# nateraw/stable-diffusion-videos

Hardware: NVIDIA H100
Metric: frames/sec at 512x512 50-step SD-1.4 (higher is better)
Workload: dtype f16

## Files before the change

### include/sdwalk.h

```cpp
#ifndef SDWALK_H_
#define SDWALK_H_

#include <stdint.h>

#ifdef __cplusplus
extern "C" {
#endif

#define SDW_ABI_VERSION 2

const char* sdw_last_error(void);
int sdw_abi_version(void);
void sdw_debug_plan_only(int on);

int sdw_slerp_lerp_batch(const void* lat_a, const void* lat_b, const void* emb_a, const void* emb_b,
                         const float* t, int n_frames, int64_t n_lat, int64_t n_emb, int dtype_is_f16,
                         float dot_threshold, void* out_lat, void* out_emb, void* stream);

typedef struct sdw_step_coef {
  float guidance;
  float c_x;
  float c_e[5];
  int32_t hist_slot[4];
  int32_t use_x_base;
// ... 61 lines not shown
int sdw_engine_debug_profile(sdw_engine* e, const char* path, void* stream);

typedef struct sdw_gemm_desc {
  const void* A;
  int32_t C, W, H, B;
  int64_t sW, sH, sB;
  int32_t conv;
  int32_t up_px, up_py;
  const void* Wt;
  int32_t N;
  int64_t ldb, Kb;
  int32_t b_batched;
  int64_t sBh, sBb;
  const float* bias;
  const float* rowvec;
  int32_t rowvec_ld;
  const void* resid;
  int64_t ldr;
  void* out;
  int64_t ldc;
  int64_t o_sW, o_sH, o_sB;
  int32_t mode;
  int32_t act;
  float alpha;
  int32_t vt_col0, vt_d, vt_heads, vt_ntok;
  void* vt;
  int64_t vt_ld;
  int32_t bn;
  int32_t ver;
  int32_t nsub;
  int32_t ew;
  int32_t tr;
  int32_t et;
  int32_t reserved0;
} sdw_gemm_desc;

int sdw_gemm(const sdw_gemm_desc* desc, void* stream);
int sdw_debug_plan(const sdw_gemm_desc* desc, int32_t out[12]);

int sdw_attention(const void* q, int64_t q_ld, const void* k, int64_t k_ld, const void* vt, int64_t vt_ld, int B,
                  int Nq, int Nk, int heads, int d, void* out, int64_t out_ld, void* stream);

int sdw_groupnorm(const void* x, int64_t ldx, int B, int64_t P, int C, int G, const float* gamma, const float* beta,
                  float eps, int silu, void* y, int64_t ldy, void* stream);
int sdw_layernorm(const void* x, int64_t ldx, int64_t rows, int C, const float* gamma, const float* beta, float eps,
                  void* y, int64_t ldy, void* stream);

int sdw_softmax_rows(void* s, int64_t ld, int64_t rows, int n, void* stream);
int sdw_conv_in_small(const void* x, int64_t ldx, int B, int H, int W, int Cin, const void* w, const float* bias, int N,
                      void* y, int64_t ldy, void* stream);
int sdw_conv_out_small(const void* x, int64_t ldx, int B, int H, int W, int C, const void* w, const float* bias, int nout,
                       float* out_f32, uint8_t* out_u8, void* stream);
int sdw_vae_in(const float* x, float inv_scale, const void* w, const float* bias, int F, int C, int H, int W, void* z,
               void* stream);
int sdw_timestep_embed(const float* t, int n, int dim, int round_f16, float* out, void* stream);
int sdw_linear_f32(const float* in, int64_t ldi, const void* w, const float* bias, int M, int N, int K, int silu_in,
                   int silu_out, float* out, int64_t ldo, void* stream);
int sdw_wrap_pad(const void* x, int64_t ld_bytes, int B, int H, int W, int pix_bytes, int pad, void* y, void* stream);
int sdw_crop_interior(const void* yp, int B, int H, int W, int pix_bytes, int crop, const void* resid_f16, int64_t ldr,
                      void* out, int64_t ldo_bytes, void* stream);

int sdw_debug_attention_plan(int B, int Nq, int Nk, int heads, int d, int32_t out[5]);

int sdw_pack_weight(const void* w_oihw, int N, int C, int kh, int kw, int geglu_interleave, void* out, void* stream);
int sdw_pack_weight_up4(const void* w_oihw, int N, int C, void* out, void* stream);

typedef struct sdw_clip sdw_clip;
// ... 54 lines not shown
```

### stable-diffusion-videos_b200/_native.py

```python
import ctypes as C
import os

import torch

_HERE = os.path.dirname(os.path.abspath(__file__))
LIB_PATH = os.path.join(_HERE, "libsdwalk.so")
_lib = None


class SdwError(RuntimeError):
    pass


class StepCoef(C.Structure):
    _fields_ = [
        ("guidance", C.c_float), ("c_x", C.c_float), ("c_e", C.c_float * 5),
        ("hist_slot", C.c_int32 * 4), ("use_x_base", C.c_int32), ("save_x_base", C.c_int32),
        ("push_slot", C.c_int32), ("next_in_scale", C.c_float), ("push_e", C.c_float), ("push_x", C.c_float),
    ]


class GemmDesc(C.Structure):
    _fields_ = [
        ("A", C.c_void_p), ("C", C.c_int32), ("W", C.c_int32), ("H", C.c_int32), ("B", C.c_int32),
        ("sW", C.c_int64), ("sH", C.c_int64), ("sB", C.c_int64),
        ("conv", C.c_int32), ("up_px", C.c_int32), ("up_py", C.c_int32),
        ("Wt", C.c_void_p), ("N", C.c_int32), ("ldb", C.c_int64), ("Kb", C.c_int64),
        ("b_batched", C.c_int32), ("sBh", C.c_int64), ("sBb", C.c_int64),
        ("bias", C.c_void_p), ("rowvec", C.c_void_p), ("rowvec_ld", C.c_int32),
        ("resid", C.c_void_p), ("ldr", C.c_int64),
        ("out", C.c_void_p), ("ldc", C.c_int64),
        ("o_sW", C.c_int64), ("o_sH", C.c_int64), ("o_sB", C.c_int64),
        ("mode", C.c_int32), ("act", C.c_int32), ("alpha", C.c_float),
        ("vt_col0", C.c_int32), ("vt_d", C.c_int32), ("vt_heads", C.c_int32), ("vt_ntok", C.c_int32),
        ("vt", C.c_void_p), ("vt_ld", C.c_int64), ("bn", C.c_int32), ("ver", C.c_int32), ("nsub", C.c_int32), ("ew", C.c_int32), ("tr", C.c_int32), ("et", C.c_int32), ("reserved0", C.c_int32),
    ]


def lib():
    global _lib
    if _lib is None:
        if not os.path.exists(LIB_PATH):
            raise SdwError(
                f"{LIB_PATH} not built: run `python __graft_entry__.py build` "
                "(the native sm_90a library is required; there is no fallback path)")
        _lib = C.CDLL(LIB_PATH)
        _lib.sdw_last_error.restype = C.c_char_p
    return _lib


def check(rc):
    if rc != 0:
        raise SdwError(f"libsdwalk error {rc}: {lib().sdw_last_error().decode()}")


def stream_ptr():
    return C.c_void_p(torch.cuda.current_stream().cuda_stream)


def ptr(t):
    return C.c_void_p(t.data_ptr()) if t is not None else C.c_void_p(0)


def require_cuda(*tensors):
    for t in tensors:
        if t is not None and not t.is_cuda:
            raise SdwError("libsdwalk operates on CUDA tensors only (no CPU fallback)")

# ... 129 lines not shown
```

### stable-diffusion-videos_b200/csrc/sdw_capi.cu

```cuda
#include "../../include/sdwalk.h"
#include "sdw_internal.h"

#include <cstdlib>
#include <cstring>

namespace sdw {
static thread_local std::string g_err;
void set_error(const std::string& msg) { g_err = msg; }
bool pdl_enabled() {
  static const bool on = [] { const char* e = std::getenv("SDW_PDL"); return e && e[0] == '1'; }();
  return on;
}
const char* last_error() { return g_err.c_str(); }
}

using namespace sdw;

extern "C" {

const char* sdw_last_error(void) { return sdw::last_error(); }
int sdw_abi_version(void) { return SDW_ABI_VERSION; }
void sdw_debug_plan_only(int on) { sdw::set_plan_only(on != 0); }

int sdw_slerp_lerp_batch(const void* lat_a, const void* lat_b, const void* emb_a, const void* emb_b, const float* t,
                         int n_frames, int64_t n_lat, int64_t n_emb, int dtype_is_f16, float dot_threshold,
                         void* out_lat, void* out_emb, void* stream) {
  return slerp_lerp_batch(lat_a, lat_b, emb_a, emb_b, t, n_frames, n_lat, n_emb, dtype_is_f16, dot_threshold,
                          out_lat, out_emb, static_cast<cudaStream_t>(stream));
}

int sdw_cfg_sched_step(const void* eps_nhwc, int has_uncond, float* x, float* x_base, float* hist,
                       const sdw_step_coef* coef, int F, int C, int H, int W, void* next_in, int next_in_cpad,
                       void* stream) {
  return cfg_sched_step(static_cast<const float*>(eps_nhwc), has_uncond, x, x_base, hist, coef, F, C, H, W, next_in,
                        next_in_cpad, static_cast<cudaStream_t>(stream));
}

int sdw_latents_init(const void* latents, int dtype_is_f16, float init_noise_sigma, float in_scale, float* x,
                     void* model_in, int model_in_cpad, int dup, int F, int C, int H, int W, void* stream) {
  return latents_init(latents, dtype_is_f16, init_noise_sigma, in_scale, x, model_in, model_in_cpad, dup, F, C, H, W,
                      static_cast<cudaStream_t>(stream));
}

static int to_desc(const sdw_gemm_desc* c, GemmDesc& d);

int sdw_debug_plan(const sdw_gemm_desc* c, int32_t out[12]) {
  SDW_REQUIRE(c != nullptr && out != nullptr, "null");
  GemmDesc d;
  if (int e = to_desc(c, d)) return e;
  GemmLaunch L;
  if (int e = plan_gemm(d, &L)) return e;
  out[0] = L.ver; out[1] = L.bn; out[2] = L.nsub; out[3] = L.ew; out[4] = L.tr;
  out[5] = L.p.epi_tma; out[6] = L.p.nstages; out[7] = 0;
  out[8] = static_cast<int32_t>(L.grid.x); out[9] = L.p.bw; out[10] = L.p.bh; out[11] = L.p.bb;
  return 0;
}

int sdw_gemm(const sdw_gemm_desc* c, void* stream) {
  SDW_REQUIRE(c != nullptr, "null desc");
  GemmDesc d;
  if (int e = to_desc(c, d)) return e;
  GemmLaunch L;
  if (int e = plan_gemm(d, &L)) return e;
  return launch_gemm(L, static_cast<cudaStream_t>(stream));
}

static int to_desc(const sdw_gemm_desc* c, GemmDesc& d) {
  d.A = static_cast<const __half*>(c->A);
  d.C = c->C; d.W = c->W; d.H = c->H; d.B = c->B;
  d.sW = c->sW; d.sH = c->sH; d.sB = c->sB;
  d.conv = c->conv; d.up_px = c->up_px; d.up_py = c->up_py;
  d.Wt = static_cast<const __half*>(c->Wt);
  d.N = c->N; d.ldb = c->ldb; d.Kb = c->Kb;
  d.b_batched = c->b_batched; d.sBh = c->sBh; d.sBb = c->sBb;
  d.bias = c->bias; d.rowvec = c->rowvec; d.rowvec_ld = c->rowvec_ld;
  d.resid = static_cast<const __half*>(c->resid); d.ldr = c->ldr;
  d.out = static_cast<__half*>(c->out); d.ldc = c->ldc;
  d.o_sW = c->o_sW; d.o_sH = c->o_sH; d.o_sB = c->o_sB;
  d.mode = c->mode; d.act = c->act; d.alpha = c->alpha;
  d.vt_col0 = c->vt_col0; d.vt_d = c->vt_d; d.vt_heads = c->vt_heads; d.vt_ntok = c->vt_ntok;
  d.vt = static_cast<__half*>(c->vt); d.vt_ld = c->vt_ld;
  d.bn = c->bn;
  d.ver = c->ver;
  d.nsub = c->nsub;
  d.ew = c->ew;
  d.tr = c->tr;
  d.et = c->et;
  return 0;
}

int sdw_attention(const void* q, int64_t q_ld, const void* k, int64_t k_ld, const void* vt, int64_t vt_ld, int B,
                  int Nq, int Nk, int heads, int d, void* out, int64_t out_ld, void* stream) {
  AttnDesc a;
  a.q = static_cast<const __half*>(q); a.q_ld = q_ld;
  a.k = static_cast<const __half*>(k); a.k_ld = k_ld;
  a.vt = static_cast<const __half*>(vt); a.vt_ld = vt_ld;
  a.B = B; a.Nq = Nq; a.Nk = Nk; a.heads = heads; a.d = d;
  a.out = static_cast<__half*>(out); a.out_ld = out_ld;
  AttnLaunch L;
  if (int e = plan_attention(a, &L)) return e;
  return launch_attention(L, static_cast<cudaStream_t>(stream));
}

int sdw_groupnorm(const void* x, int64_t ldx, int B, int64_t P, int C, int G, const float* gamma, const float* beta,
                  float eps, int silu, void* y, int64_t ldy, void* stream) {
  cudaStream_t st = static_cast<cudaStream_t>(stream);
  float2* ws = nullptr;
  SDW_CUDA_OK(cudaMallocAsync(&ws, gn_workspace_bytes(B), st));
  const int rc = groupnorm(static_cast<const __half*>(x), ldx, B, P, C, G, gamma, beta, eps, silu, static_cast<__half*>(y),
                           ldy, ws, st);
  cudaFreeAsync(ws, st);
  return rc;
}

int sdw_layernorm(const void* x, int64_t ldx, int64_t rows, int C, const float* gamma, const float* beta, float eps,
                  void* y, int64_t ldy, void* stream) {
  return layernorm(static_cast<const __half*>(x), ldx, rows, C, gamma, beta, eps, static_cast<__half*>(y), ldy,
                   static_cast<cudaStream_t>(stream));
}

// ... 67 lines not shown
```

### stable-diffusion-videos_b200/csrc/sdw_gemm.cu

```cuda
#include "sdw_internal.h"
#include "sdw_ptx.cuh"

#include <cudaTypedefs.h>

#include <algorithm>
#include <cstdlib>
#include <cstring>

namespace sdw {

static constexpr int BM = 128;
static constexpr int BK = 64;
static constexpr int GEMM_THREADS = 288;
static constexpr int A_STAGE = BM * BK * 2;
static constexpr int TR_BW = 16, TR_BH = 8;
static constexpr int A_STAGE_TR = (TR_BH + 2) * TR_BW * 128;

template <int BN, int NSUB, int TR>
struct GemmCfg {
  static constexpr int A_BYTES = TR ? A_STAGE_TR : A_STAGE;
  static constexpr int TAPS = TR ? 3 : 1;
  static constexpr int B_SUB = BN * 128;
  static constexpr int B_BYTES = TAPS * NSUB * B_SUB;
};

struct EpiRow {
  bool ok;
  int64_t out_off, res_off, pix;
  const float* rowvec;
};

template <int BN, int XE>
__device__ __forceinline__ void gemm_epilogue(const GemmKParams& p, float (&acc)[BN / 2], int n_base, const EpiRow (&R)[2],
                                              int lane, int wg, int lrow0, uint8_t* stage, uint64_t* res_full, int x0,
                                              int y0, int b0, uint32_t& chunk_count) {
  const int q2 = 2 * (lane & 3);
  const bool vec2 = p.vec2;
  const bool use_tma = p.epi_tma;
  const int r0 = 64 * wg;
  const int tx = x0 + (r0 & (p.bw - 1)), ty = y0 + ((r0 >> p.lg_bw) & (p.bh - 1)), tb = b0 + (r0 >> (p.lg_bw + p.lg_bh));
  const bool issuer = (threadIdx.x & 127) == 0;
  const bool tma_res = use_tma && p.resid != nullptr;
  const int nch = (min(BN, p.N - n_base) + 31) >> 5;
  auto res_issue = [&](int c, uint32_t k) {
    if (tma_res && issuer && c < nch) {
      mbar_expect_tx(&res_full[k & 1], 4096);
      tma_load_4d(&p.mapRes, &res_full[k & 1], stage + (k & 1) * 4096, n_base + 32 * c, tx, ty, tb);
    }
  };
  if (tma_res && p.mode == GEMM_PLAIN) {
    if (issuer) bulk_wait_group_read<1>();
    res_issue(0, chunk_count);
  }

  auto value = [&](float v, int n, int h) {
    float o = v * p.alpha;
    if (p.bias) o += __ldg(p.bias + n);
    if (p.rowvec) o += __ldg(R[h].rowvec + n);
    if (p.act == 1) o = silu_f(o);
    if constexpr (XE != 0) {
      if (p.act == 2) o = o > 0.f ? o : 0.2f * o;
    }
    return o;
  };
  auto add_res = [&](float& o, float r) {
    if constexpr (XE != 0) o = fmaf(p.res_scale, r, o);
    else o += r;
  };
  auto plain_pair = [&](int j, int n, uint8_t* staged, int scol) {
#pragma unroll
    for (int h = 0; h < 2; ++h) {
      float o0 = n < p.N ? value(acc[4 * j + 2 * h], n, h) : 0.f;
// ... 9 lines not shown
          add_res(o0, f.x);
          add_res(o1, f.y);
          if (XE != 0 && p.resid2) {
            const float2 g = __half22float2(*reinterpret_cast<const __half2*>(p.resid2 + R[h].res_off + n));
            o0 += g.x;
            o1 += g.y;
          }
        } else {
          if (n < p.N) add_res(o0, __half2float(p.resid[R[h].res_off + n]));
          if (n + 1 < p.N) add_res(o1, __half2float(p.resid[R[h].res_off + n + 1]));
          if (XE != 0 && p.resid2) {
            if (n < p.N) o0 += __half2float(p.resid2[R[h].res_off + n]);
            if (n + 1 < p.N) o1 += __half2float(p.resid2[R[h].res_off + n + 1]);
          }
        }
      }
      if (staged) {
        *reinterpret_cast<uint32_t*>(staged + (lrow0 + 8 * h) * 64 + scol * 2) = pack_h2(o0, o1);
      } else if (R[h].ok) {
        __half* dst = p.out + R[h].out_off + n;
        if (vec2 && n + 1 < p.N) {
          *reinterpret_cast<uint32_t*>(dst) = pack_h2(o0, o1);
        } else {
          if (n < p.N) dst[0] = __float2half_rn(o0);
          if (n + 1 < p.N) dst[1] = __float2half_rn(o1);
        }
      }
    }
  };
  auto vt_pair = [&](int j, int n) {
#pragma unroll
    for (int h = 0; h < 2; ++h) {
      if (!R[h].ok) continue;
      const int64_t bq = R[h].pix / p.vt_ntok;
      const int tok = static_cast<int>(R[h].pix - bq * p.vt_ntok);
#pragma unroll
      for (int e = 0; e < 2; ++e) {
        const int nn = n + e;
        if (nn >= p.N) continue;
        float o = acc[4 * j + 2 * h + e] * p.alpha;
        if (p.bias) o += __ldg(p.bias + nn);
        const int cc = nn - p.vt_col0, head = cc / p.vt_d, dd = cc - head * p.vt_d;
        p.vt[((bq * p.vt_heads + head) * p.vt_d + dd) * p.vt_ld + tok] = __float2half_rn(o);
      }
    }
  };
  auto stage_begin = [&]() {
    if (issuer) bulk_wait_group_read<1>();
    asm volatile("bar.sync %0, 128;" ::"r"(1 + wg) : "memory");
    return stage + (chunk_count & 1) * 4096;
  };
  auto stage_end = [&](uint8_t* buf, int col) {
    fence_proxy_async_smem();
    asm volatile("bar.sync %0, 128;" ::"r"(1 + wg) : "memory");
    if (issuer) {
      tma_store_4d(&p.mapOut, buf, col, tx, ty, tb);
      bulk_commit_group();
    }
    ++chunk_count;
  };

  if (p.mode == GEMM_GEGLU) {
#pragma unroll
    for (int c = 0; c < BN / 64; ++c) {
      const int n = n_base + 64 * c;
      if (n >= p.N) break;
      uint8_t* buf = use_tma ? stage_begin() : nullptr;
#pragma unroll
      for (int jj = 0; jj < 4; ++jj) {
        const int j = 8 * c + jj;
        const int na = n + 8 * jj + q2, ng = na + 32;
        float o[2][2];
#pragma unroll
        for (int h = 0; h < 2; ++h)
#pragma unroll
          for (int e = 0; e < 2; ++e) {
// ... 20 lines not shown
          }
        }
      }
      if (use_tma) stage_end(buf, n / 2);
    }
    return;
  }
#pragma unroll
  for (int c = 0; c < BN / 32; ++c) {
    const int n = n_base + 32 * c;
    if (n >= p.N) break;
    if (p.mode == GEMM_QKV_VT && n >= p.vt_col0) {
#pragma unroll
      for (int jj = 0; jj < 4; ++jj) vt_pair(4 * c + jj, n + 8 * jj + q2);
      continue;
    }
    if (use_tma) {
      uint8_t* buf = stage_begin();
      if (tma_res) {
        if (issuer && c + 1 < nch) bulk_wait_group_read<0>();
        res_issue(c + 1, chunk_count + 1);
        mbar_wait(&res_full[chunk_count & 1], (chunk_count >> 1) & 1);
      }
#pragma unroll
      for (int jj = 0; jj < 4; ++jj) plain_pair(4 * c + jj, n + 8 * jj + q2, buf, 8 * jj + q2);
      stage_end(buf, n);
    } else {
#pragma unroll
      for (int jj = 0; jj < 4; ++jj) plain_pair(4 * c + jj, n + 8 * jj + q2, nullptr, 0);
    }
  }
}

template <int BN, int NSUB, int TR, int CL, int XE>
__global__ void __launch_bounds__(GEMM_THREADS, 1) gemm_kernel(const __grid_constant__ GemmKParams p) {
  using Cfg = GemmCfg<BN, NSUB, TR>;
  constexpr int A_BYTES = Cfg::A_BYTES;
  constexpr int B_BYTES = Cfg::B_BYTES;
  const int STAGES = p.nstages;
  extern __shared__ uint8_t smem_raw[];
  uint8_t* smem = reinterpret_cast<uint8_t*>((reinterpret_cast<uintptr_t>(smem_raw) + 1023) & ~uintptr_t(1023));
  uint64_t* full_bar = reinterpret_cast<uint64_t*>(smem);
  uint64_t* empty_bar = full_bar + GEMM_MAX_STAGES;
  uint8_t* smem_a = smem + GEMM_BAR_BYTES;
  uint8_t* smem_b = smem_a + STAGES * A_BYTES;
  uint8_t* epi_stage = smem_b + STAGES * B_BYTES;
  uint64_t* res_full = empty_bar + GEMM_MAX_STAGES;

  const int warp = threadIdx.x >> 5, lane = threadIdx.x & 31;
  const uint32_t rank = CL > 1 ? cluster_ctarank() : 0;
  const int cluster_id = blockIdx.x / CL;
  const int nclusters = gridDim.x / CL;
  const int total_tiles = p.m_groups * p.n_tiles;
  const int num_kb = TR ? 3 * p.kchunks : p.ntaps * p.kchunks;

  if (warp == 8 && lane == 0) {
    tma_prefetch_desc(&p.mapA[0]);
    tma_prefetch_desc(&p.mapB);
    if (p.epi_tma) tma_prefetch_desc(&p.mapOut);
    for (int s = 0; s < STAGES; ++s) {
      mbar_init(&full_bar[s], 1);
      mbar_init(&empty_bar[s], 2 * CL);
    }
    for (int i = 0; i < 4; ++i) mbar_init(&res_full[i], 1);
    if (p.epi_tma && p.resid) tma_prefetch_desc(&p.mapRes);
    fence_barrier_init();
  }
  if (CL > 1) cluster_sync_all();
  else __syncthreads();
  pdl_wait();
  pdl_launch_dependents();

  auto tile_coords = [&](int t, int& x0, int& y0, int& b0, int& n0) {
    const int m_group = t / p.n_tiles;
    const int n_tile = t - m_group * p.n_tiles;
    const int m_tile = m_group * CL + static_cast<int>(rank);
    const int twh = p.tiles_w * p.tiles_h;
    const int tb = m_tile / twh;
    const int rem = m_tile - tb * twh;
    const int th = rem / p.tiles_w;
    const int tw = rem - th * p.tiles_w;
    x0 = tw * p.bw;
    y0 = th * p.bh;
    b0 = tb * p.bb;
    n0 = n_tile * (NSUB * BN);
  };

  if (warp == 8) {
    if (lane == 0) {
      int stage = 0;
      uint32_t phase = 0;
      for (int t = cluster_id; t < total_tiles; t += nclusters) {
        int x0, y0, b0, n0;
        tile_coords(t, x0, y0, b0, n0);
        int tap = 0, kc = 0;
        for (int kb = 0; kb < num_kb; ++kb) {
          mbar_wait(&empty_bar[stage], phase ^ 1);
          mbar_expect_tx(&full_bar[stage], A_BYTES + B_BYTES);
          uint8_t* a_dst = smem_a + stage * A_BYTES;
          uint8_t* b_dst = smem_b + stage * B_BYTES + rank * (BN / CL) * 128;
          const int nrow = n0 + static_cast<int>(rank) * (BN / CL);
          if (TR) {
            const int kx = tap;
            tma_load_4d(&p.mapA[0], &full_bar[stage], a_dst, kc * BK, x0 + kx - 1, y0 - 1, b0);
          } else {
            tma_load_4d(&p.mapA[p.tap_map[tap]], &full_bar[stage], a_dst, kc * BK, x0 + p.tap_dx[tap], y0 + p.tap_dy[tap],
                        b0);
          }
#pragma unroll
          for (int ky = 0; ky < Cfg::TAPS; ++ky)
#pragma unroll
            for (int sub = 0; sub < NSUB; ++sub) {
              const int kcoord = TR ? ((ky * 3 + tap) * p.kchunks + kc) * BK : kb * BK;
              uint8_t* dst = b_dst + (ky * NSUB + sub) * Cfg::B_SUB;
              const int c2 = p.b_batched ? y0 : 0, c3 = p.b_batched ? b0 : 0;
              if (CL > 1)
                tma_load_4d_mc(&p.mapB, &full_bar[stage], dst, kcoord, nrow + sub * BN, c2, c3, (1u << CL) - 1);
              else
                tma_load_4d(&p.mapB, &full_bar[stage], dst, kcoord, nrow + sub * BN, c2, c3);
            }
          if (++stage == STAGES) {
            stage = 0;
            phase ^= 1;
          }
          if (TR) {
            if (++tap == 3) {
              tap = 0;
              ++kc;
            }
          } else if (++kc == p.kchunks) {
            kc = 0;
            ++tap;
          }
        }
      }
    }
  } else {
    const int wg = warp >> 2;
    const int lrow0 = 16 * (warp & 3) + (lane >> 2);
    uint8_t* stage_buf = epi_stage + wg * 8192;
    uint32_t chunk_count = 0;
    auto release = [&](int s) {
      if ((threadIdx.x & 127) == 0) {
        if (CL > 1) {
#pragma unroll
          for (int r = 0; r < CL; ++r) mbar_arrive_cluster(mapa_rank(smem_u32(&empty_bar[s]), r));
        } else {
          mbar_arrive(&empty_bar[s]);
        }
      }
    };
    int stage = 0;
    uint32_t phase = 0;
    float acc[NSUB][BN / 2];
    for (int t = cluster_id; t < total_tiles; t += nclusters) {
      int x0, y0, b0, n0;
      tile_coords(t, x0, y0, b0, n0);
#pragma unroll
      for (int sub = 0; sub < NSUB; ++sub)
#pragma unroll
        for (int i = 0; i < BN / 2; ++i) acc[sub][i] = 0.f;
      int prev = -1;
      for (int kb = 0; kb < num_kb; ++kb) {
        mbar_wait(&full_bar[stage], phase);
        const uint32_t a_base = smem_u32(smem_a + stage * A_BYTES);
        const uint32_t b_base = smem_u32(smem_b + stage * B_BYTES);
        wgmma_fence();
#pragma unroll
        for (int ky = 0; ky < Cfg::TAPS; ++ky) {
          const uint32_t a_off = TR ? (4 * wg + ky) * (TR_BW * 128) : wg * (64 * 128);
          const uint64_t da = make_desc_k_sw128(a_base + a_off);
#pragma unroll
          for (int k = 0; k < BK / 16; ++k)
#pragma unroll
            for (int sub = 0; sub < NSUB; ++sub) {
              const uint64_t db = make_desc_k_sw128(b_base + (ky * NSUB + sub) * Cfg::B_SUB);
              Wgmma<BN>::ss(acc[sub], da + 2 * k, db + 2 * k, (kb | ky | k) != 0 ? 1u : 0u);
            }
        }
        wgmma_commit();
        wgmma_wait<1>();
        if (prev >= 0) release(prev);
        prev = stage;
        if (++stage == STAGES) {
          stage = 0;
          phase ^= 1;
        }
      }
      wgmma_wait<0>();
#pragma unroll
      for (int sub = 0; sub < NSUB; ++sub) reg_fence(acc[sub]);
      release(prev);

      EpiRow R[2];
#pragma unroll
      for (int h = 0; h < 2; ++h) {
        const int r = 64 * wg + lrow0 + 8 * h;
        const int x = x0 + (r & (p.bw - 1)), y = y0 + ((r >> p.lg_bw) & (p.bh - 1)), b = b0 + (r >> (p.lg_bw + p.lg_bh));
        R[h].ok = x < p.W && y < p.H && b < p.B;
        R[h].pix = (static_cast<int64_t>(b) * p.H + y) * p.W + x;
        const int64_t oyy = static_cast<int64_t>(y) * p.os + p.oy, oxx = static_cast<int64_t>(x) * p.os + p.ox;
        R[h].out_off = static_cast<int64_t>(b) * p.o_sB + oyy * p.o_sH + oxx * p.o_sW;
        R[h].res_off = static_cast<int64_t>(b) * p.r_sB + oyy * p.r_sH + oxx * p.r_sW;
        R[h].rowvec = p.rowvec ? p.rowvec + static_cast<int64_t>(b) * p.rowvec_ld : nullptr;
      }
#pragma unroll
      for (int sub = 0; sub < NSUB; ++sub)
        gemm_epilogue<BN, XE>(p, acc[sub], n0 + sub * BN, R, lane, wg, lrow0, stage_buf, res_full + 2 * wg, x0, y0, b0,
                          chunk_count);
    }
    if (p.epi_tma && (threadIdx.x & 127) == 0) bulk_wait_group<0>();
  }

  if (CL > 1) cluster_sync_all();
}

static PFN_cuTensorMapEncodeTiled_v12000 g_encode = nullptr;
static bool g_plan_only = false;
void set_plan_only(bool on) { g_plan_only = on; }

int sm_count() {
  static int n = 0;
  if (g_plan_only) return H100_SMS;
  if (n == 0) {
    int dev = 0;
    if (cudaGetDevice(&dev) != cudaSuccess || cudaDeviceGetAttribute(&n, cudaDevAttrMultiProcessorCount, dev) != cudaSuccess ||
        n <= 0) {
      (void)cudaGetLastError();
      n = H100_SMS;
    }
  }
  return n;
}

int gemm_init() {
  if (g_encode || g_plan_only) return 0;
  void* fn = nullptr;
  cudaDriverEntryPointQueryResult qres;
  SDW_CUDA_OK(cudaGetDriverEntryPoint("cuTensorMapEncodeTiled", &fn, cudaEnableDefault, &qres));
  if (qres != cudaDriverEntryPointSuccess || !fn) {
    set_error("cuTensorMapEncodeTiled driver entry point not available");
    return 2;
// ... 203 lines not shown
    const int groups = (m_tiles_f + CL - 1) / CL;
    for (int i = 0; i < 4; ++i) {
      const int c = cand[i];
      if (d.mode == GEMM_GEGLU && c % 64 != 0) continue;
      if (stages_for(c, 1, reuse, epi_bytes) < 2) continue;
      const int tiles = groups * ((d.N + c - 1) / c);
      const int waves = (tiles + nsm / CL - 1) / (nsm / CL);
      double cost = static_cast<double>(waves) * c;
      if (stages_for(c, 1, reuse, epi_bytes) < 3) cost *= 1.6;
      if (cost < best) {
        best = cost;
        bn = c;
      }
    }
  }
  SDW_REQUIRE(bn == 32 || bn == 64 || bn == 128 || bn == 160 || bn == 256 || (bn == 192 && ver == 2), "unsupported BLOCK_N");
  if (ver == 2) SDW_REQUIRE(bn != 32 && bn != 64, "the CTA-pair kernel needs BLOCK_N >= 128");
  if (d.ew == 4) SDW_REQUIRE(false, "one epilogue form on this GPU: epilogue width 4 is not available");
  SDW_REQUIRE(d.ew == 0 || d.ew == 2, "epilogue width must be 0 (auto) or 2");
  L->ew = 2;
  L->ver = ver;
  L->nsub = nsub;
  L->bn = bn;
  if (d.mode == GEMM_GEGLU) SDW_REQUIRE(bn % 64 == 0 && d.N % 64 == 0, "GEGLU needs 64-column pairs");
  if (d.mode == GEMM_QKV_VT) SDW_REQUIRE(d.vt && d.vt_col0 % 32 == 0 && d.vt_d > 0, "bad V^T split");
  p.nstages = stages_for(bn, nsub, reuse, epi_bytes);
  SDW_REQUIRE(p.nstages >= 2, "no room for a two-stage operand pipeline");
  p.m_groups = (m_tiles_f + CL - 1) / CL;
  p.n_tiles = (d.N + bn * nsub - 1) / (bn * nsub);
  {
    const int64_t total = static_cast<int64_t>(p.m_groups) * p.n_tiles;
    SDW_REQUIRE(total < (int64_t(1) << 31), "tile grid too large");
    L->grid = dim3(static_cast<unsigned>(CL * std::min<int64_t>(total, nsm / CL)), 1, 1);
  }
  {
    auto lg2 = [](int v) { int l = 0; while ((1 << l) < v) ++l; return l; };
    p.lg_bw = lg2(p.bw);
    p.lg_bh = lg2(p.bh);
    SDW_REQUIRE((1 << p.lg_bw) == p.bw && (1 << p.lg_bh) == p.bh, "tile extents must be powers of two");
  }
  for (int m = 0; m < nmaps; ++m) {
    const __half* base = d.A;
    uint64_t dims[4] = {static_cast<uint64_t>(d.C), static_cast<uint64_t>(d.W), static_cast<uint64_t>(d.H),
                        static_cast<uint64_t>(d.B)};
    uint64_t strides[4] = {1, static_cast<uint64_t>(d.sW), static_cast<uint64_t>(d.sH), static_cast<uint64_t>(d.sB)};
    if (d.conv == 2) {
      const int py = m / 2, px = m % 2;
      base = d.A + py * d.sH + px * d.sW;
      dims[1] = Wd;
      dims[2] = Hd;
      strides[1] = 2 * d.sW;
      strides[2] = 2 * d.sH;
    }
    for (int i = 1; i < 4; ++i)
      if (strides[i] == 0) strides[i] = static_cast<uint64_t>(Cp);
    uint32_t box[4] = {BK, static_cast<uint32_t>(bw), static_cast<uint32_t>(reuse ? bh + 2 : bh), static_cast<uint32_t>(bb)};
    if (int e = encode_map(&p.mapA[m], base, 4, dims, strides, box)) return e;
  }
  {
    const int64_t ldb = d.ldb ? d.ldb : static_cast<int64_t>(p.ntaps) * Cp;
    uint64_t dims[4] = {static_cast<uint64_t>(d.Kb ? d.Kb : static_cast<int64_t>(p.ntaps) * Cp),
                        static_cast<uint64_t>(d.N), static_cast<uint64_t>(d.b_batched ? Hd : 1),
                        static_cast<uint64_t>(d.b_batched ? d.B : 1)};
    uint64_t strides[4] = {1, static_cast<uint64_t>(ldb), static_cast<uint64_t>(d.b_batched ? d.sBh : 0),
                           static_cast<uint64_t>(d.b_batched ? d.sBb : 0)};
    for (int i = 2; i < 4; ++i)
// ... 16 lines not shown
      for (int i = 2; i < 4; ++i)
        if (sr[i] == 0 || sr[i] % 8 != 0) sr[i] = sr[1] * static_cast<uint64_t>(Wd);
      if (int e = encode_map(&p.mapRes, d.resid + p.oy * res_sH + p.ox * res_sW, 4, dims, sr, box, 0)) return e;
    }
  }
  p.bias = d.bias;
  p.rowvec = d.rowvec;
  p.rowvec_ld = d.rowvec_ld;
  p.resid = d.resid;
  p.res_scale = d.res_scale;
  p.resid2 = d.resid2;
  p.out = d.out;
  p.o_sW = osW;
  p.o_sH = osH;
  p.o_sB = osB;
  p.r_sW = res_sW;
  p.r_sH = res_sH;
  p.r_sB = res_sB;
  p.vec2 = ((p.o_sW | p.o_sH | p.o_sB) & 1) == 0 && (reinterpret_cast<uintptr_t>(d.out) & 3) == 0 &&
           (!d.resid || (((p.r_sW | p.r_sH | p.r_sB) & 1) == 0 && (reinterpret_cast<uintptr_t>(d.resid) & 3) == 0)) &&
           (!d.resid2 || (reinterpret_cast<uintptr_t>(d.resid2) & 3) == 0);
  p.mode = d.mode;
  p.act = d.act;
  p.alpha = d.alpha;
  p.vt_col0 = d.vt_col0;
  p.vt_d = d.vt_d;
  p.vt_heads = d.vt_heads;
  p.vt_ntok = d.vt_ntok > 0 ? d.vt_ntok : 1;
  p.vt = d.vt;
  p.vt_ld = d.vt_ld;
  return 0;
}

template <int BN, int NSUB, int TR, int CL, int XE = 0>
static int launch_one(const GemmLaunch& l, cudaStream_t stream) {
  static int max_ctas = 0;
  if (!max_ctas) {
    SDW_CUDA_OK(cudaFuncSetAttribute(gemm_kernel<BN, NSUB, TR, CL, XE>, cudaFuncAttributeMaxDynamicSharedMemorySize,
                                     GEMM_SMEM_DYN));
    max_ctas = sm_count();
    if (CL > 1) {
      cudaLaunchConfig_t cfg{};
      cfg.gridDim = dim3(CL * (sm_count() / CL));
      cfg.blockDim = dim3(GEMM_THREADS);
      cfg.dynamicSmemBytes = GEMM_SMEM_DYN;
      cudaLaunchAttribute attr[1];
      attr[0].id = cudaLaunchAttributeClusterDimension;
      attr[0].val.clusterDim.x = CL;
      attr[0].val.clusterDim.y = 1;
      attr[0].val.clusterDim.z = 1;
      cfg.attrs = attr;
      cfg.numAttrs = 1;
      int nclusters = 0;
      SDW_CUDA_OK(cudaOccupancyMaxActiveClusters(&nclusters, gemm_kernel<BN, NSUB, TR, CL, XE>, &cfg));
      if (nclusters > 0) max_ctas = std::min(max_ctas, CL * nclusters);
    }
  }
  const dim3 grid(std::min<unsigned>(l.grid.x, static_cast<unsigned>(max_ctas)), 1, 1);
  SDW_CUDA_OK(launch_cluster(gemm_kernel<BN, NSUB, TR, CL, XE>, grid, dim3(GEMM_THREADS), GEMM_SMEM_DYN, stream, CL, l.p));
  SDW_CUDA_OK(cudaGetLastError());
  return 0;
}

int launch_gemm(const GemmLaunch& l, cudaStream_t stream) {
  const int key = l.xe * 1000000 + l.ver * 100000 + l.bn * 100 + l.nsub * 10 + (l.tr ? 1 : 0);
  switch (key) {
    case 1103210: return launch_one<32, 1, 0, 1, 1>(l, stream);
    case 1106410: return launch_one<64, 1, 0, 1, 1>(l, stream);
    case 106410: return launch_one<64, 1, 0, 1>(l, stream);
    case 112810: return launch_one<128, 1, 0, 1>(l, stream);
    case 116010: return launch_one<160, 1, 0, 1>(l, stream);
    case 125610: return launch_one<256, 1, 0, 1>(l, stream);
    case 212810: return launch_one<128, 1, 0, 2>(l, stream);
    case 216010: return launch_one<160, 1, 0, 2>(l, stream);
    case 219210: return launch_one<192, 1, 0, 2>(l, stream);
    case 225610: return launch_one<256, 1, 0, 2>(l, stream);
    case 216020: return launch_one<160, 2, 0, 2>(l, stream);
    case 212811: return launch_one<128, 1, 1, 2>(l, stream);
    case 216011: return launch_one<160, 1, 1, 2>(l, stream);
    case 219211: return launch_one<192, 1, 1, 2>(l, stream);
    case 225611: return launch_one<256, 1, 1, 2>(l, stream);
    case 216021: return launch_one<160, 2, 1, 2>(l, stream);
    default: break;
  }
  set_error("no GEMM kernel for this version / BLOCK_N / accumulators / tap reuse combination");
  return 1;
}

}
```

### stable-diffusion-videos_b200/csrc/sdw_internal.h

```cpp
#pragma once
#include <cuda.h>
#include <cuda_fp16.h>
#include <cuda_runtime.h>
#include <stdint.h>

#include <cstdio>
#include <functional>
#include <string>
#include <unordered_map>
#include <vector>

namespace sdw {

void set_error(const std::string& msg);
const char* last_error();
#define SDW_CUDA_OK(expr)                                                                      \
  do {                                                                                         \
    cudaError_t _e = (expr);                                                                   \
    if (_e != cudaSuccess) {                                                                   \
      (void)cudaGetLastError();  \
      ::sdw::set_error(std::string(#expr) + ": " + cudaGetErrorString(_e));                    \
      return 2;                                                                                \
    }                                                                                          \
  } while (0)
// ... 69 lines not shown
  int m_groups, n_tiles;
  int N;
  int b_batched;
  int epi_tma;
  int nstages;
  int vec2;
  const float* bias;
  const float* rowvec;
  int rowvec_ld;
  const __half* resid;
  int64_t r_sW, r_sH, r_sB;
  float res_scale;
  const __half* resid2;
  __half* out;
  int64_t o_sW, o_sH, o_sB;
  int os, ox, oy;
  int mode;
  int act;
  float alpha;
  int vt_col0, vt_d, vt_heads, vt_ntok;
  __half* vt;
  int64_t vt_ld;
};

struct GemmLaunch {
  GemmKParams p;
  dim3 grid;
  int bn;
  int ver;
  int nsub = 1;
  int ew = 2;
  int tr = 0;
  int xe = 0;
};

struct GemmDesc {
  const __half* A = nullptr;
  int C = 0, W = 0, H = 1, B = 1;
  int64_t sW = 0, sH = 0, sB = 0;
  int conv = 0;
  int up_px = 0, up_py = 0;
  const __half* Wt = nullptr;
  int N = 0;
  int64_t ldb = 0;
  int64_t Kb = 0;
  int b_batched = 0;
  int64_t sBh = 0, sBb = 0;
  const float* bias = nullptr;
  const float* rowvec = nullptr;
  int rowvec_ld = 0;
  const __half* resid = nullptr;
  int64_t ldr = 0;
  int64_t r_sW = 0, r_sH = 0, r_sB = 0;
  float res_scale = 1.f;
  const __half* resid2 = nullptr;
  __half* out = nullptr;
  int64_t ldc = 0;
  int64_t o_sW = 0, o_sH = 0, o_sB = 0;
  int mode = GEMM_PLAIN;
  int act = 0;
  float alpha = 1.f;
  int vt_col0 = 0, vt_d = 0, vt_heads = 0, vt_ntok = 0;
  __half* vt = nullptr;
  int64_t vt_ld = 0;
  int bn = 0;
  int ver = 0;
  int nsub = 0;
  int ew = 0;
  int tr = 0;
  int et = 0;
};

int plan_gemm(const GemmDesc& d, GemmLaunch* out);
int launch_gemm(const GemmLaunch& l, cudaStream_t stream);
void set_plan_only(bool on);
int gemm_init();
constexpr int GEMM_SMEM_DYN = 227 * 1024;
constexpr int GEMM_SMEM_USABLE = GEMM_SMEM_DYN - 1024;
constexpr int GEMM_BAR_BYTES = 1024;
constexpr int GEMM_MAX_STAGES = 8;
constexpr int GEMM_EPI_BYTES = 2 * 2 * 4096;
int encode_map(CUtensorMap* map, const void* base, int rank, const uint64_t* dims, const uint64_t* strides_elems,
               const uint32_t* box, int swizzle_bytes = 128);

struct AttnDesc {
  const __half* q = nullptr;
  int64_t q_ld = 0;
  const __half* k = nullptr;
  int64_t k_ld = 0;
  const __half* vt = nullptr;
  int64_t vt_ld = 0;
  int B = 0, Nq = 0, Nk = 0, heads = 0, d = 0;
  __half* out = nullptr;
  int64_t out_ld = 0;
};
struct AttnLaunch {
  alignas(64) unsigned char storage[704];
};
bool attn_supported(int d);
int plan_attention(const AttnDesc& a, AttnLaunch* L);
int launch_attention(const AttnLaunch& L, cudaStream_t stream);
void attention_plan_info(const AttnLaunch& L, int out[5]);

// ... 107 lines not shown
```

Measured before the change: 3.062.

## Add ping-pong warpgroup schedule to the persistent TMA/WGMMA GEMM kernel

Adds a ping-pong schedule in which two consumer warpgroups each own a whole 128-row tile and alternate their mainloops through named barriers, so one warpgroup's epilogue overlaps the other's tensor-core work. The kernel grows to 384 threads with setmaxnreg splitting registers between producer and consumers, and the QKV-transposed epilogue precomputes per-row offsets to drop the per-element divisions. The planner picks ping-pong automatically for BLOCK_N 128/160 single-accumulator GEMMs with long K loops and more tiles than CTAs. Each consumer now keeps two full accumulators, which raises register pressure, and the barrier ordering could stall or stay unbalanced when the tile count is odd.

```diff
diff --git a/include/sdwalk.h b/include/sdwalk.h
--- a/include/sdwalk.h
+++ b/include/sdwalk.h
@@ -117,7 +117,7 @@
   int32_t ew;
   int32_t tr;
   int32_t et;
-  int32_t reserved0;
+  int32_t sched;
 } sdw_gemm_desc;
 
 int sdw_gemm(const sdw_gemm_desc* desc, void* stream);
diff --git a/stable-diffusion-videos_b200/_native.py b/stable-diffusion-videos_b200/_native.py
--- a/stable-diffusion-videos_b200/_native.py
+++ b/stable-diffusion-videos_b200/_native.py
@@ -33,7 +33,7 @@
         ("o_sW", C.c_int64), ("o_sH", C.c_int64), ("o_sB", C.c_int64),
         ("mode", C.c_int32), ("act", C.c_int32), ("alpha", C.c_float),
         ("vt_col0", C.c_int32), ("vt_d", C.c_int32), ("vt_heads", C.c_int32), ("vt_ntok", C.c_int32),
-        ("vt", C.c_void_p), ("vt_ld", C.c_int64), ("bn", C.c_int32), ("ver", C.c_int32), ("nsub", C.c_int32), ("ew", C.c_int32), ("tr", C.c_int32), ("et", C.c_int32), ("reserved0", C.c_int32),
+        ("vt", C.c_void_p), ("vt_ld", C.c_int64), ("bn", C.c_int32), ("ver", C.c_int32), ("nsub", C.c_int32), ("ew", C.c_int32), ("tr", C.c_int32), ("et", C.c_int32), ("sched", C.c_int32),
     ]
 
 
diff --git a/stable-diffusion-videos_b200/csrc/sdw_capi.cu b/stable-diffusion-videos_b200/csrc/sdw_capi.cu
--- a/stable-diffusion-videos_b200/csrc/sdw_capi.cu
+++ b/stable-diffusion-videos_b200/csrc/sdw_capi.cu
@@ -51,7 +51,7 @@
   GemmLaunch L;
   if (int e = plan_gemm(d, &L)) return e;
   out[0] = L.ver; out[1] = L.bn; out[2] = L.nsub; out[3] = L.ew; out[4] = L.tr;
-  out[5] = L.p.epi_tma; out[6] = L.p.nstages; out[7] = 0;
+  out[5] = L.p.epi_tma; out[6] = L.p.nstages; out[7] = L.pp ? 2 : 1;
   out[8] = static_cast<int32_t>(L.grid.x); out[9] = L.p.bw; out[10] = L.p.bh; out[11] = L.p.bb;
   return 0;
 }
@@ -86,6 +86,7 @@
   d.ew = c->ew;
   d.tr = c->tr;
   d.et = c->et;
+  d.sched = c->sched;
   return 0;
 }
 
diff --git a/stable-diffusion-videos_b200/csrc/sdw_gemm.cu b/stable-diffusion-videos_b200/csrc/sdw_gemm.cu
--- a/stable-diffusion-videos_b200/csrc/sdw_gemm.cu
+++ b/stable-diffusion-videos_b200/csrc/sdw_gemm.cu
@@ -11,7 +11,10 @@
 
 static constexpr int BM = 128;
 static constexpr int BK = 64;
-static constexpr int GEMM_THREADS = 288;
+static constexpr int GEMM_THREADS = 384;
+static constexpr int GEMM_PRODUCER_REGS = 40;
+static constexpr int GEMM_CONSUMER_REGS = 232;
+static constexpr int GEMM_BAR_PINGPONG = 3;
 static constexpr int A_STAGE = BM * BK * 2;
 static constexpr int TR_BW = 16, TR_BH = 8;
 static constexpr int A_STAGE_TR = (TR_BH + 2) * TR_BW * 128;
@@ -26,18 +29,19 @@
 
 struct EpiRow {
   bool ok;
-  int64_t out_off, res_off, pix;
+  int64_t out_off, res_off;
+  int64_t vt_off;
   const float* rowvec;
 };
 
 template <int BN, int XE>
 __device__ __forceinline__ void gemm_epilogue(const GemmKParams& p, float (&acc)[BN / 2], int n_base, const EpiRow (&R)[2],
-                                              int lane, int wg, int lrow0, uint8_t* stage, uint64_t* res_full, int x0,
-                                              int y0, int b0, uint32_t& chunk_count) {
+                                              int lane, int wg, int half, int lrow0, uint8_t* stage, uint64_t* res_full,
+                                              int x0, int y0, int b0, uint32_t& chunk_count) {
   const int q2 = 2 * (lane & 3);
   const bool vec2 = p.vec2;
   const bool use_tma = p.epi_tma;
-  const int r0 = 64 * wg;
+  const int r0 = 64 * half;
   const int tx = x0 + (r0 & (p.bw - 1)), ty = y0 + ((r0 >> p.lg_bw) & (p.bh - 1)), tb = b0 + (r0 >> (p.lg_bw + p.lg_bh));
   const bool issuer = (threadIdx.x & 127) == 0;
   const bool tma_res = use_tma && p.resid != nullptr;
@@ -113,16 +117,13 @@
 #pragma unroll
     for (int h = 0; h < 2; ++h) {
       if (!R[h].ok) continue;
-      const int64_t bq = R[h].pix / p.vt_ntok;
-      const int tok = static_cast<int>(R[h].pix - bq * p.vt_ntok);
 #pragma unroll
       for (int e = 0; e < 2; ++e) {
         const int nn = n + e;
         if (nn >= p.N) continue;
         float o = acc[4 * j + 2 * h + e] * p.alpha;
         if (p.bias) o += __ldg(p.bias + nn);
-        const int cc = nn - p.vt_col0, head = cc / p.vt_d, dd = cc - head * p.vt_d;
-        p.vt[((bq * p.vt_heads + head) * p.vt_d + dd) * p.vt_ld + tok] = __float2half_rn(o);
+        p.vt[R[h].vt_off + static_cast<int64_t>(nn - p.vt_col0) * p.vt_ld] = __float2half_rn(o);
       }
     }
   };
@@ -209,8 +210,9 @@
   }
 }
 
-template <int BN, int NSUB, int TR, int CL, int XE>
+template <int BN, int NSUB, int TR, int CL, int XE, int PP>
 __global__ void __launch_bounds__(GEMM_THREADS, 1) gemm_kernel(const __grid_constant__ GemmKParams p) {
+  static_assert(!PP || (NSUB == 1 && XE == 0 && (BN == 128 || BN == 160)), "ping-pong: one accumulator, BLOCK_N 128 / 160");
   using Cfg = GemmCfg<BN, NSUB, TR>;
   constexpr int A_BYTES = Cfg::A_BYTES;
   constexpr int B_BYTES = Cfg::B_BYTES;
@@ -237,7 +239,7 @@
     if (p.epi_tma) tma_prefetch_desc(&p.mapOut);
     for (int s = 0; s < STAGES; ++s) {
       mbar_init(&full_bar[s], 1);
-      mbar_init(&empty_bar[s], 2 * CL);
+      mbar_init(&empty_bar[s], (PP ? 1 : 2) * CL);
     }
     for (int i = 0; i < 4; ++i) mbar_init(&res_full[i], 1);
     if (p.epi_tma && p.resid) tma_prefetch_desc(&p.mapRes);
@@ -263,8 +265,9 @@
     n0 = n_tile * (NSUB * BN);
   };
 
-  if (warp == 8) {
-    if (lane == 0) {
+  if (warp >= 8) {
+    setmaxnreg_dec<GEMM_PRODUCER_REGS>();
+    if (warp == 8 && lane == 0) {
       int stage = 0;
       uint32_t phase = 0;
       for (int t = cluster_id; t < total_tiles; t += nclusters) {
@@ -313,6 +316,7 @@
       }
     }
   } else {
+    setmaxnreg_inc<GEMM_CONSUMER_REGS>();
     const int wg = warp >> 2;
     const int lrow0 = 16 * (warp & 3) + (lane >> 2);
     uint8_t* stage_buf = epi_stage + wg * 8192;
@@ -329,14 +333,32 @@
     };
     int stage = 0;
     uint32_t phase = 0;
-    float acc[NSUB][BN / 2];
-    for (int t = cluster_id; t < total_tiles; t += nclusters) {
+    auto skip_tile = [&]() {
+      const int s = stage + num_kb;
+      phase ^= static_cast<uint32_t>(s / STAGES) & 1u;
+      stage = s % STAGES;
+    };
+    constexpr int NACC = PP ? 2 : NSUB;
+    auto acc_half = [&](int i) { return PP ? i : wg; };
+    auto acc_sub = [&](int i) { return PP ? 0 : i; };
+    float acc[NACC][BN / 2];
+    const uint32_t bar_mine = GEMM_BAR_PINGPONG + wg, bar_other = GEMM_BAR_PINGPONG + (wg ^ 1);
+    int t = cluster_id;
+    if (PP) {
+      if (wg == 1) {
+        if (t < total_tiles) named_bar_arrive(GEMM_BAR_PINGPONG, 256);
+        t += nclusters;
+        skip_tile();
+      }
+    }
+    for (; t < total_tiles; t += (PP ? 2 : 1) * nclusters) {
       int x0, y0, b0, n0;
       tile_coords(t, x0, y0, b0, n0);
 #pragma unroll
-      for (int sub = 0; sub < NSUB; ++sub)
-#pragma unroll
-        for (int i = 0; i < BN / 2; ++i) acc[sub][i] = 0.f;
+      for (int i = 0; i < NACC; ++i)
+#pragma unroll
+        for (int j = 0; j < BN / 2; ++j) acc[i][j] = 0.f;
+      if (PP) named_bar_sync(bar_mine, 256);
       int prev = -1;
       for (int kb = 0; kb < num_kb; ++kb) {
         mbar_wait(&full_bar[stage], phase);
@@ -345,14 +367,14 @@
         wgmma_fence();
 #pragma unroll
         for (int ky = 0; ky < Cfg::TAPS; ++ky) {
-          const uint32_t a_off = TR ? (4 * wg + ky) * (TR_BW * 128) : wg * (64 * 128);
-          const uint64_t da = make_desc_k_sw128(a_base + a_off);
 #pragma unroll
           for (int k = 0; k < BK / 16; ++k)
 #pragma unroll
-            for (int sub = 0; sub < NSUB; ++sub) {
-              const uint64_t db = make_desc_k_sw128(b_base + (ky * NSUB + sub) * Cfg::B_SUB);
-              Wgmma<BN>::ss(acc[sub], da + 2 * k, db + 2 * k, (kb | ky | k) != 0 ? 1u : 0u);
+            for (int i = 0; i < NACC; ++i) {
+              const uint32_t a_off = TR ? (4 * acc_half(i) + ky) * (TR_BW * 128) : acc_half(i) * (64 * 128);
+              const uint64_t da = make_desc_k_sw128(a_base + a_off);
+              const uint64_t db = make_desc_k_sw128(b_base + (ky * NSUB + acc_sub(i)) * Cfg::B_SUB);
+              Wgmma<BN>::ss(acc[i], da + 2 * k, db + 2 * k, (kb | ky | k) != 0 ? 1u : 0u);
             }
         }
         wgmma_commit();
@@ -364,27 +386,35 @@
           phase ^= 1;
         }
       }
+      if (PP && t + nclusters < total_tiles) named_bar_arrive(bar_other, 256);
       wgmma_wait<0>();
 #pragma unroll
-      for (int sub = 0; sub < NSUB; ++sub) reg_fence(acc[sub]);
+      for (int i = 0; i < NACC; ++i) reg_fence(acc[i]);
       release(prev);
-
-      EpiRow R[2];
-#pragma unroll
-      for (int h = 0; h < 2; ++h) {
-        const int r = 64 * wg + lrow0 + 8 * h;
-        const int x = x0 + (r & (p.bw - 1)), y = y0 + ((r >> p.lg_bw) & (p.bh - 1)), b = b0 + (r >> (p.lg_bw + p.lg_bh));
-        R[h].ok = x < p.W && y < p.H && b < p.B;
-        R[h].pix = (static_cast<int64_t>(b) * p.H + y) * p.W + x;
-        const int64_t oyy = static_cast<int64_t>(y) * p.os + p.oy, oxx = static_cast<int64_t>(x) * p.os + p.ox;
-        R[h].out_off = static_cast<int64_t>(b) * p.o_sB + oyy * p.o_sH + oxx * p.o_sW;
-        R[h].res_off = static_cast<int64_t>(b) * p.r_sB + oyy * p.r_sH + oxx * p.r_sW;
-        R[h].rowvec = p.rowvec ? p.rowvec + static_cast<int64_t>(b) * p.rowvec_ld : nullptr;
-      }
-#pragma unroll
-      for (int sub = 0; sub < NSUB; ++sub)
-        gemm_epilogue<BN, XE>(p, acc[sub], n0 + sub * BN, R, lane, wg, lrow0, stage_buf, res_full + 2 * wg, x0, y0, b0,
-                          chunk_count);
+      if (PP) skip_tile();
+
+#pragma unroll
+      for (int i = 0; i < NACC; ++i) {
+        const int half = acc_half(i);
+        EpiRow R[2];
+#pragma unroll
+        for (int h = 0; h < 2; ++h) {
+          const int r = 64 * half + lrow0 + 8 * h;
+          const int x = x0 + (r & (p.bw - 1)), y = y0 + ((r >> p.lg_bw) & (p.bh - 1)), b = b0 + (r >> (p.lg_bw + p.lg_bh));
+          R[h].ok = x < p.W && y < p.H && b < p.B;
+          if (p.mode == GEMM_QKV_VT) {
+            const int64_t pix = (static_cast<int64_t>(b) * p.H + y) * p.W + x;
+            const int64_t bq = pix / p.vt_ntok;
+            R[h].vt_off = bq * p.vt_heads * p.vt_d * p.vt_ld + (pix - bq * p.vt_ntok);
+          }
+          const int64_t oyy = static_cast<int64_t>(y) * p.os + p.oy, oxx = static_cast<int64_t>(x) * p.os + p.ox;
+          R[h].out_off = static_cast<int64_t>(b) * p.o_sB + oyy * p.o_sH + oxx * p.o_sW;
+          R[h].res_off = static_cast<int64_t>(b) * p.r_sB + oyy * p.r_sH + oxx * p.r_sW;
+          R[h].rowvec = p.rowvec ? p.rowvec + static_cast<int64_t>(b) * p.rowvec_ld : nullptr;
+        }
+        gemm_epilogue<BN, XE>(p, acc[i], n0 + acc_sub(i) * BN, R, lane, wg, half, lrow0, stage_buf, res_full + 2 * wg,
+                              x0, y0, b0, chunk_count);
+      }
     }
     if (p.epi_tma && (threadIdx.x & 127) == 0) bulk_wait_group<0>();
   }
@@ -654,6 +684,13 @@
     const int64_t total = static_cast<int64_t>(p.m_groups) * p.n_tiles;
     SDW_REQUIRE(total < (int64_t(1) << 31), "tile grid too large");
     L->grid = dim3(static_cast<unsigned>(CL * std::min<int64_t>(total, nsm / CL)), 1, 1);
+    SDW_REQUIRE(d.sched >= 0 && d.sched <= 2, "schedule: 0 auto, 1 cooperative, 2 ping-pong");
+    const bool pp_ok = (bn == 128 || bn == 160) && nsub == 1 && !xe;
+    if (d.sched == 2)
+      SDW_REQUIRE(pp_ok && total >= 2, "the ping-pong schedule needs BLOCK_N 128 or 160, one accumulator, no extended "
+                                       "epilogue and at least two tiles");
+    const int num_kb = reuse ? 3 * kchunks : p.ntaps * kchunks;
+    L->pp = d.sched == 2 || (d.sched == 0 && pp_ok && total > L->grid.x / CL && num_kb >= 60) ? 1 : 0;
   }
   {
     auto lg2 = [](int v) { int l = 0; while ((1 << l) < v) ++l; return l; };
@@ -736,11 +773,11 @@
   return 0;
 }
 
-template <int BN, int NSUB, int TR, int CL, int XE = 0>
+template <int BN, int NSUB, int TR, int CL, int XE = 0, int PP = 0>
 static int launch_one(const GemmLaunch& l, cudaStream_t stream) {
   static int max_ctas = 0;
   if (!max_ctas) {
-    SDW_CUDA_OK(cudaFuncSetAttribute(gemm_kernel<BN, NSUB, TR, CL, XE>, cudaFuncAttributeMaxDynamicSharedMemorySize,
+    SDW_CUDA_OK(cudaFuncSetAttribute(gemm_kernel<BN, NSUB, TR, CL, XE, PP>, cudaFuncAttributeMaxDynamicSharedMemorySize,
                                      GEMM_SMEM_DYN));
     max_ctas = sm_count();
     if (CL > 1) {
@@ -756,19 +793,25 @@
       cfg.attrs = attr;
       cfg.numAttrs = 1;
       int nclusters = 0;
-      SDW_CUDA_OK(cudaOccupancyMaxActiveClusters(&nclusters, gemm_kernel<BN, NSUB, TR, CL, XE>, &cfg));
+      SDW_CUDA_OK(cudaOccupancyMaxActiveClusters(&nclusters, gemm_kernel<BN, NSUB, TR, CL, XE, PP>, &cfg));
       if (nclusters > 0) max_ctas = std::min(max_ctas, CL * nclusters);
     }
   }
   const dim3 grid(std::min<unsigned>(l.grid.x, static_cast<unsigned>(max_ctas)), 1, 1);
-  SDW_CUDA_OK(launch_cluster(gemm_kernel<BN, NSUB, TR, CL, XE>, grid, dim3(GEMM_THREADS), GEMM_SMEM_DYN, stream, CL, l.p));
+  SDW_CUDA_OK(launch_cluster(gemm_kernel<BN, NSUB, TR, CL, XE, PP>, grid, dim3(GEMM_THREADS), GEMM_SMEM_DYN, stream, CL, l.p));
   SDW_CUDA_OK(cudaGetLastError());
   return 0;
 }
 
 int launch_gemm(const GemmLaunch& l, cudaStream_t stream) {
-  const int key = l.xe * 1000000 + l.ver * 100000 + l.bn * 100 + l.nsub * 10 + (l.tr ? 1 : 0);
+  const int key = l.pp * 10000000 + l.xe * 1000000 + l.ver * 100000 + l.bn * 100 + l.nsub * 10 + (l.tr ? 1 : 0);
   switch (key) {
+    case 10112810: return launch_one<128, 1, 0, 1, 0, 1>(l, stream);
+    case 10116010: return launch_one<160, 1, 0, 1, 0, 1>(l, stream);
+    case 10212810: return launch_one<128, 1, 0, 2, 0, 1>(l, stream);
+    case 10216010: return launch_one<160, 1, 0, 2, 0, 1>(l, stream);
+    case 10212811: return launch_one<128, 1, 1, 2, 0, 1>(l, stream);
+    case 10216011: return launch_one<160, 1, 1, 2, 0, 1>(l, stream);
     case 1103210: return launch_one<32, 1, 0, 1, 1>(l, stream);
     case 1106410: return launch_one<64, 1, 0, 1, 1>(l, stream);
     case 106410: return launch_one<64, 1, 0, 1>(l, stream);
@@ -787,7 +830,7 @@
     case 216021: return launch_one<160, 2, 1, 2>(l, stream);
     default: break;
   }
-  set_error("no GEMM kernel for this version / BLOCK_N / accumulators / tap reuse combination");
+  set_error("no GEMM kernel for this version / BLOCK_N / accumulators / tap reuse / schedule combination");
   return 1;
 }
 
diff --git a/stable-diffusion-videos_b200/csrc/sdw_internal.h b/stable-diffusion-videos_b200/csrc/sdw_internal.h
--- a/stable-diffusion-videos_b200/csrc/sdw_internal.h
+++ b/stable-diffusion-videos_b200/csrc/sdw_internal.h
@@ -125,6 +125,7 @@
   int ew = 2;
   int tr = 0;
   int xe = 0;
+  int pp = 0;
 };
 
 struct GemmDesc {
@@ -162,6 +163,7 @@
   int ew = 0;
   int tr = 0;
   int et = 0;
+  int sched = 0;
 };
 
 int plan_gemm(const GemmDesc& d, GemmLaunch* out);
```

New measurement: 3.092 (median of 6 runs). About the same (+1.0%).
